# meffmadd/intro-tc-vae

Hardware: AMD Instinct MI355X
Metric: images/sec (64x64x3, z=128, bs=64) intro-TC step (higher is better)
Workload: dtype f32 in/out/accumulate, conv products on split-fp16 MFMA (two scaled fp16 planes, 3 products, fp32-class)

## Files before the change

### intro-tc-vae_amd/csrc/abi.hip

```cpp
#include "conv_shared.h"

#include <vector>

namespace itcv {
thread_local char g_err[512] = "";

struct ProfRec {
  int code;
  double flop;
  hipEvent_t start, stop;
};
static bool g_prof_on = false;
static std::vector<ProfRec> g_prof;

static thread_local int g_prof_depth = 0;
ProfScope::ProfScope(hipStream_t stream, int kind, int ks, int bm, int up2, int ns, double flop) : st(stream), slot(-1) {
  if (++g_prof_depth > 1 || !g_prof_on) return;
  ProfRec r;
  r.code = kind | (ks << 4) | (bm << 8) | (up2 << 16) | (ns << 20);
  r.flop = flop;
  if (hipEventCreate(&r.start) != hipSuccess || hipEventCreate(&r.stop) != hipSuccess) return;
  g_prof.push_back(r);
  slot = (int)g_prof.size() - 1;
  g_prof_start = r.start, g_prof_stop = r.stop;
}
ProfScope::~ProfScope() {
  if (--g_prof_depth > 0) return;
  if (slot >= 0 && g_prof_start) {
    (void)hipEventDestroy(g_prof[slot].start);
    (void)hipEventDestroy(g_prof[slot].stop);
    g_prof.pop_back();
  }
  g_prof_start = g_prof_stop = nullptr;
}
thread_local hipEvent_t g_prof_start = nullptr, g_prof_stop = nullptr;
Options g_opt;
}

extern "C" {
int itcv_abi_version(void) { return ITCV_ABI_VERSION; }

int itcv_set_option(const char* name, int value) {
  if (!name) return itcv::fail("%s: null option name", "itcv_set_option");
  if (!strcmp(name, "band_m16")) {
    if (value != 0 && value != 1) return itcv::fail("%s: band_m16 takes 0 or 1 (got %lld)", "itcv_set_option", value);
    itcv::g_opt.band_m16 = value;
    return 0;
  }
  if (!strcmp(name, "band_persist_blocks")) {
    if (value < 0 || value > 1024) return itcv::fail("%s: band_persist_blocks takes 0..1024 (got %lld)", "itcv_set_option", value);
    itcv::g_opt.band_persist_blocks = value;
    return 0;
  }
  if (!strcmp(name, "wgrad_m16")) {
    if (value != 0 && value != 1) return itcv::fail("%s: wgrad_m16 takes 0 or 1 (got %lld)", "itcv_set_option", value);
    itcv::g_opt.wgrad_m16 = value;
    return 0;
  }
  if (!strcmp(name, "planes_mfma_waves")) {
    if (value != 4 && value != 8) return itcv::fail("%s: planes_mfma_waves takes 4 or 8 (got %lld)", "itcv_set_option", value);
    itcv::g_opt.planes_mfma_waves = value;
    return 0;
  }
  return itcv::fail("%s: unknown option", "itcv_set_option");
}
int itcv_get_option(const char* name) {
  if (name && !strcmp(name, "band_m16")) return itcv::g_opt.band_m16;
  if (name && !strcmp(name, "band_persist_blocks")) return itcv::g_opt.band_persist_blocks;
  if (name && !strcmp(name, "wgrad_m16")) return itcv::g_opt.wgrad_m16;
  if (name && !strcmp(name, "planes_mfma_waves")) return itcv::g_opt.planes_mfma_waves;
  return -1;
}
const char* itcv_last_error(void) { return itcv::g_err; }

int itcv_profile_begin(void) {
  itcv::g_prof.clear();
  itcv::g_prof_on = true;
  return 0;
}
int itcv_profile_end(void) {
  itcv::g_prof_on = false;
  for (auto& r : itcv::g_prof) (void)hipEventSynchronize(r.stop);
  return (int)itcv::g_prof.size();
}
int itcv_profile_get(int i, int* code, double* flop, float* ms) {
  if (i < 0 || i >= (int)itcv::g_prof.size()) return itcv::fail("%s: index out of range", "itcv_profile_get");
  const auto& r = itcv::g_prof[i];
  *code = r.code;
  *flop = r.flop;
  if (hipEventElapsedTime(ms, r.start, r.stop) != hipSuccess) *ms = -1.f;
  return 0;
}
int itcv_profile_clear(void) {
  for (auto& r : itcv::g_prof) {
    (void)hipEventDestroy(r.start);
    (void)hipEventDestroy(r.stop);
  }
  itcv::g_prof.clear();
  return 0;
}
}
```

### intro-tc-vae_amd/csrc/conv_shared.h

```cpp
#pragma once
#include <stdlib.h>

#include "common.h"

namespace itcv {

#ifdef ITCV_DIAG
#define ITCV_ABL(args, bits) (((args).ablate & (bits)) != 0)
#define ITCV_DBG(args) ((args).debug != 0)
static int diag_ablate() {
  static int v = -1;
  if (v < 0) {
    const char* e = getenv("ITCV_ABLATE");
    v = e ? atoi(e) : 0;
  }
  return v;
}
#else
#define ITCV_ABL(args, bits) (false)
#define ITCV_DBG(args) (false)
#endif

typedef float f32x16 __attribute__((ext_vector_type(16)));
typedef float f32x4_t __attribute__((ext_vector_type(4)));
typedef float f32x4 __attribute__((ext_vector_type(4)));

#pragma clang diagnostic ignored "-Winline-asm"
__device__ __forceinline__ void lds_dma16(const void* gptr, uint32_t lds_base) {
  asm volatile("s_mov_b32 m0, %0\n\ts_nop 0\n\tglobal_load_lds_dwordx4 %1, off"
               :
               : "s"(__builtin_amdgcn_readfirstlane(lds_base)), "v"(gptr)
               : "memory", "m0");
}
__device__ __forceinline__ uint32_t lds_addr(const void* p) {
  return (uint32_t)(size_t)(const __attribute__((address_space(3))) void*)p;
}
template <int N>
__device__ __forceinline__ void wait_vmcnt() {
  asm volatile("s_waitcnt vmcnt(%0)" ::"n"(N) : "memory");
}

static inline int log2_exact(int v) {
  if (v <= 0 || (v & (v - 1))) return -1;
  int s = 0;
  while ((1 << s) < v) ++s;
  return s;
}

struct ConvArgsP2 {
  const u32x4* xp;
  const u32x4* wp;
  const float* bias;
  float* y;
  int B, Ci, H, Co;
  int Mp, N;
  int mt, nt;
  int cpt, cpt_per_split;
  int SR, NSEG, NP, NPC, PXB;
  int h_shift;
  float* stats;
  int stat_T;
  const ScaleRec* xscale;
  size_t slab_stride, plane_stride;
#ifdef ITCV_DIAG
  int debug;
#endif
};

__host__ __device__ constexpr int band_taps_per_stage(int bm, int bn, int ) {
  return (bm == 64 || bn == 128) ? 2 : 1;
}

template <bool M16, bool F16 = false>
struct BandMfma;
template <bool F16>
struct BandMfma<false, F16> {
  typedef f32x16 acc_t;
  static constexpr int TS = 32, NR = 16, KSN = 2;
  static __device__ __forceinline__ acc_t mma(bf16x8 a, bf16x8 b, acc_t c) { return mma32x32x16<F16>(a, b, c); }
  static __device__ __forceinline__ int row(int r, int kq) { return (r & 3) + 8 * (r >> 2) + 4 * kq; }
};
template <bool F16>
struct BandMfma<true, F16> {
  typedef float acc_t __attribute__((ext_vector_type(4)));
  static constexpr int TS = 16, NR = 4, KSN = 1;
  static __device__ __forceinline__ acc_t mma(bf16x8 a, bf16x8 b, acc_t c) { return mma16x16x32<F16>(a, b, c); }
  static __device__ __forceinline__ int row(int r, int kq) { return 4 * kq + r; }
};

struct Options {
  int band_m16 = 1;
  int band_persist_blocks = 256;
  int wgrad_m16 = 1;
  int planes_mfma_waves = 8;
};
extern Options g_opt;
inline int band_m16() { return g_opt.band_m16; }

struct FwdPlanP2 {
  int ok, bm, bn, mt, nt, cpt, splits, cps, SR, NSEG, NP, NPC, PXB;
  int rows2;
  size_t lds;
};

FwdPlanP2 plan_fwd_p2(int B, int Ci, int H, int W, int Co, int KS, int ns);
void launch_fwd_p2(const ConvArgsP2& a, const FwdPlanP2& p, int W, int up2, int f16, hipStream_t st);
bool band_is_persistent(const ConvArgsP2& a, const FwdPlanP2& p);

}
```

### intro-tc-vae_amd/csrc/norm_act.hip

```cpp
#include <stdlib.h>

#include "common.h"

namespace itcv {

constexpr int kRedThreads = 256;

__device__ __forceinline__ uint32_t fdiv(uint32_t a, uint32_t d, int sh) { return sh >= 0 ? (a >> sh) : (a / d); }

struct BnGrp {
  size_t xs;
  size_t os;
  size_t dys;
  size_t ps;
  int cs;
  int G;
};

struct BnFinal {
  double count;
  float eps, momentum;
  float* running_mean;
  float* running_var;
  int64_t* nbt;
  float* mean;
  float* rstd;
};

template <bool FUSED>
__global__ __launch_bounds__(kRedThreads) void bn_moments_partial(const float* __restrict__ x,
                                                                  double* __restrict__ part, int B, int C, int HW,
                                                                  int splits, int hw_shift, BnFinal f, BnGrp grp) {
  __shared__ double scratch[kRedThreads / 64];
  const uint32_t c = blockIdx.x, s = blockIdx.y, hw_n = HW, total = (uint32_t)B * hw_n;
  const uint32_t chunk = ((total + splits - 1) / splits + 3) & ~3u;
  const uint32_t beg = s * chunk, end = min(beg + chunk, total);
  const int ngroups = (FUSED && grp.G > 1) ? grp.G : 1;
  if (!FUSED) {
    x += (size_t)blockIdx.z * grp.xs;
    part += (size_t)blockIdx.z * splits * 2 * C;
  }
 for (int gi = 0; gi < ngroups; ++gi, x += grp.xs, f.mean += grp.cs, f.rstd += grp.cs) {
  double s1 = 0.0, s2 = 0.0;
  if ((HW & 3) == 0) {
#pragma unroll 4
    for (uint32_t i = beg + threadIdx.x * 4; i < end; i += kRedThreads * 4) {
      const uint32_t b = fdiv(i, hw_n, hw_shift), hw = i - b * hw_n;
      const float4 v = *reinterpret_cast<const float4*>(x + ((size_t)b * C + c) * hw_n + hw);
      s1 += ((double)v.x + (double)v.y) + ((double)v.z + (double)v.w);
      s2 += ((double)v.x * v.x + (double)v.y * v.y) + ((double)v.z * v.z + (double)v.w * v.w);
    }
  } else {
    for (uint32_t i = beg + threadIdx.x; i < end; i += kRedThreads) {
      const uint32_t b = fdiv(i, hw_n, hw_shift), hw = i - b * hw_n;
      const float v = x[((size_t)b * C + c) * hw_n + hw];
      s1 += (double)v;
      s2 += (double)v * v;
    }
  }
  s1 = block_sum(s1, scratch);
  s2 = block_sum(s2, scratch);
  if (threadIdx.x == 0) {
    if (FUSED) {
      const double m = s1 / f.count;
      double var = s2 / f.count - m * m;
      if (var < 0.0) var = 0.0;
      f.mean[c] = (float)m;
      f.rstd[c] = (float)(1.0 / sqrt(var + (double)f.eps));
      if (f.running_mean) f.running_mean[c] = (1.f - f.momentum) * f.running_mean[c] + f.momentum * (float)m;
      if (f.running_var) {
        const double unbiased = f.count > 1.0 ? var * f.count / (f.count - 1.0) : var;
        f.running_var[c] = (1.f - f.momentum) * f.running_var[c] + f.momentum * (float)unbiased;
      }
      if (c == 0 && f.nbt) f.nbt[0] += 1;
    } else {
      part[((size_t)s * 2 + 0) * C + c] = s1;
      part[((size_t)s * 2 + 1) * C + c] = s2;
    }
  }
 }
}

__global__ void combine_partials(const double* __restrict__ part, double* __restrict__ sums, int C2, int splits) {
  const int i = blockIdx.x * blockDim.x + threadIdx.x;
  if (i >= C2) return;
// ... 254 lines not shown
                if (vg < 0.0) vg = 0.0;
              }
              if (st.running_mean) st.running_mean[c] = (1.f - st.momentum) * st.running_mean[c] + st.momentum * (float)mg;
              if (st.running_var) {
                const double unbiased = st.count > 1.0 ? vg * st.count / (st.count - 1.0) : vg;
                st.running_var[c] = (1.f - st.momentum) * st.running_var[c] + st.momentum * (float)unbiased;
              }
            }
            if (c == 0 && st.nbt) st.nbt[0] += G;
          }
        }
      }
      __syncthreads();
    }
    if (idx >= total) continue;
    const uint32_t bc8 = idx / per_plane, pp = idx - bc8 * per_plane;
    const uint32_t b = bc8 / C8, c8 = bc8 - b * C8;
    float o[8][PX];
    float4 xin[POOL ? 1 : 8];
    float p_ga[8], p_be[8], p_mu[8], p_rs[8];
#pragma unroll
    for (int j = 0; j < 8; ++j) {
      const int c = c8 * 8 + j;
      if (POOL == 0) xin[POOL ? 0 : j] = *reinterpret_cast<const float4*>(x + ((size_t)b * C + c) * HW + (size_t)pp * 4);
      p_ga[j] = gamma[c], p_be[j] = beta[c];
      p_mu[j] = STATS ? s_mean[(bc8 - g0) * 8 + j] : mean[c], p_rs[j] = STATS ? s_rstd[(bc8 - g0) * 8 + j] : rstd[c];
    }
#pragma unroll
    for (int j = 0; j < 8; ++j) {
      const int c = c8 * 8 + j;
      const float mu = p_mu[j], rs = p_rs[j];
      const float sc = p_ga[j] * rs, sh = p_be[j] - mu * sc;
      const size_t bc = (size_t)b * C + c;
      if (POOL == 0) {
        const size_t i = bc * HW + (size_t)pp * 4;
        float4 v = xin[POOL ? 0 : j];
        v.x = v.x * sc + sh, v.y = v.y * sc + sh, v.z = v.z * sc + sh, v.w = v.w * sc + sh;
        if (skip) {
          const float4 k = *reinterpret_cast<const float4*>(skip + i);
          v.x += k.x, v.y += k.y, v.z += k.z, v.w += k.w;
        }
        v.x = lrelu(v.x, slope), v.y = lrelu(v.y, slope), v.z = lrelu(v.z, slope), v.w = lrelu(v.w, slope);
        if (y) *reinterpret_cast<float4*>(y + i) = v;
        o[j][0] = v.x, o[j][1] = v.y, o[j][POOL ? 0 : 2] = v.z, o[j][POOL ? 1 : 3] = v.w;
      } else {
        const uint32_t ho = (pp * 2) / Wo, wo = pp * 2 - ho * Wo;
        const size_t src = bc * HW + (size_t)(2 * ho) * W + 2 * wo;
        const float4 a = *reinterpret_cast<const float4*>(x + src);
        const float4 bb = *reinterpret_cast<const float4*>(x + src + W);
        float v0 = a.x * sc + sh, v1 = a.y * sc + sh, v2 = bb.x * sc + sh, v3 = bb.y * sc + sh;
        float w0 = a.z * sc + sh, w1 = a.w * sc + sh, w2 = bb.z * sc + sh, w3 = bb.w * sc + sh;
        if (skip) {
          const float4 ka = *reinterpret_cast<const float4*>(skip + src);
          const float4 kb = *reinterpret_cast<const float4*>(skip + src + W);
          v0 += ka.x, v1 += ka.y, v2 += kb.x, v3 += kb.y;
          w0 += ka.z, w1 += ka.w, w2 += kb.z, w3 += kb.w;
        }
        const float r0 = 0.25f * (lrelu(v0, slope) + lrelu(v1, slope) + lrelu(v2, slope) + lrelu(v3, slope));
        const float r1 = 0.25f * (lrelu(w0, slope) + lrelu(w1, slope) + lrelu(w2, slope) + lrelu(w3, slope));
        if (y) *reinterpret_cast<float2*>(y + bc * HWo + (size_t)pp * 2) = make_float2(r0, r1);
        o[j][0] = r0, o[j][1] = r1;
      }
    }
    u32x4 chk[PX][NS];
#pragma unroll
    for (int px = 0; px < PX; ++px) {
      float v8[8];
#pragma unroll
      for (int j = 0; j < 8; ++j) v8[j] = o[j][px];
      split8<NS, F16>(v8, chk[px]);
    }
    const uint32_t cidx0 = base + (threadIdx.x & ~63u);
    if (STRIP && cidx0 + 64 <= total) {
      store_planes_wave<PX, NS>(planes, plane_stride, per_plane, (uint32_t)HWo, cidx0, chk, strips[STRIP ? threadIdx.x >> 6 : 0]);
    } else {
#pragma unroll
      for (int px = 0; px < PX; ++px)
#pragma unroll
        for (int p = 0; p < NS; ++p) planes[(size_t)p * plane_stride + (size_t)bc8 * HWo + (size_t)pp * PX + px] = chk[px][p];
    }
  }
}

template <int MODE>
__device__ __forceinline__ float upstream(const float* __restrict__ dy, size_t bc, int h, int w, int H, int W) {
  if (MODE == 0) return dy[bc * H * W + (size_t)h * W + w];
  if (MODE == 1) return 0.25f * dy[bc * (H / 2) * (W / 2) + (size_t)(h >> 1) * (W / 2) + (w >> 1)];
  const size_t base = bc * (size_t)(4 * H * W) + (size_t)(2 * h) * (2 * W) + 2 * w;
  const float2 a = *reinterpret_cast<const float2*>(dy + base);
  const float2 b = *reinterpret_cast<const float2*>(dy + base + 2 * W);
  return (a.x + a.y) + (b.x + b.y);
}

template <int MODE>
__global__ __launch_bounds__(kRedThreads) void bn_bwd_partial(const float* __restrict__ x,
                                                              const float* __restrict__ dy,
                                                              const float* __restrict__ mean,
                                                              const float* __restrict__ rstd,
                                                              const float* __restrict__ gamma,
                                                              const float* __restrict__ beta,
                                                              const float* __restrict__ skip,
                                                              double* __restrict__ part, int B, int C, int H, int W,
                                                              float slope, int splits) {
  __shared__ double scratch[kRedThreads / 64];
  const int c = blockIdx.x, s = blockIdx.y, HW = H * W;
  const size_t total = (size_t)B * HW;
  const size_t chunk = (total + splits - 1) / splits;
  const size_t beg = (size_t)s * chunk, end = beg + chunk < total ? beg + chunk : total;
  const float mu = mean[c], rs = rstd[c], ga = gamma[c], be = beta[c];
  double s1 = 0.0, s2 = 0.0;
  for (size_t i = beg + threadIdx.x; i < end; i += kRedThreads) {
    const size_t b = i / HW;
    const int hw = (int)(i - b * HW), h = hw / W, w = hw - h * W;
    const size_t bc = b * C + c;
    const float xh = (x[bc * HW + hw] - mu) * rs;
    float u = xh * ga + be;
    if (skip) u += skip[bc * HW + hw];
    float g = upstream<MODE>(dy, bc, h, w, H, W);
    if (!(u > 0.f)) g *= slope;
    s1 += (double)g;
    s2 += (double)g * (double)xh;
  }
  s1 = block_sum(s1, scratch);
  s2 = block_sum(s2, scratch);
  if (threadIdx.x == 0) {
    part[((size_t)s * 2 + 0) * C + c] = s1;
    part[((size_t)s * 2 + 1) * C + c] = s2;
  }
}

template <int MODE>
__global__ void bn_bwd_apply_kernel(const float* __restrict__ x, const float* __restrict__ dy,
                                    const float* __restrict__ mean, const float* __restrict__ rstd,
                                    const float* __restrict__ gamma, const float* __restrict__ beta,
                                    const float* __restrict__ skip, const double* __restrict__ dsums, double count,
                                    float* __restrict__ dx, float* __restrict__ dskip, int C, int H, int W,
                                    size_t n, float slope) {
  const int HW = H * W;
  for (size_t i = (size_t)blockIdx.x * blockDim.x + threadIdx.x; i < n; i += (size_t)gridDim.x * blockDim.x) {
    const size_t bc = i / HW;
    const int hw = (int)(i - bc * HW), h = hw / W, w = hw - h * W;
    const int c = (int)(bc % C);
    const float mu = mean[c], rs = rstd[c], ga = gamma[c];
    const float xh = (x[i] - mu) * rs;
    float u = xh * ga + beta[c];
    if (skip) u += skip[i];
    float g = upstream<MODE>(dy, bc, h, w, H, W);
    if (!(u > 0.f)) g *= slope;
    const float m1 = (float)(dsums[c] / count), m2 = (float)(dsums[C + c] / count);
    dx[i] = ga * rs * (g - m1 - xh * m2);
    if (dskip) dskip[i] = g;
  }
}



template <int MODE>
__device__ __forceinline__ float4 upstream4(const float* __restrict__ dy, uint32_t bc, uint32_t h, uint32_t w,
                                            uint32_t H, uint32_t W) {
  if (MODE == 0) return *reinterpret_cast<const float4*>(dy + (size_t)bc * H * W + h * W + w);
  if (MODE == 1) {
    const float2 d = *reinterpret_cast<const float2*>(dy + (size_t)bc * (H / 2) * (W / 2) + (h >> 1) * (W / 2) + (w >> 1));
    return make_float4(0.25f * d.x, 0.25f * d.x, 0.25f * d.y, 0.25f * d.y);
  }
  const float* p = dy + (size_t)bc * (4 * H * W) + (size_t)(2 * h) * (2 * W) + 2 * w;
  const float4 a0 = *reinterpret_cast<const float4*>(p), a1 = *reinterpret_cast<const float4*>(p + 4);
// ... 563 lines not shown
    ITCV_BWD_PARTIAL(1);
  else if (up2)
    ITCV_BWD_PARTIAL(2);
  else
    ITCV_BWD_PARTIAL(0);
#undef ITCV_BWD_PARTIAL
  ITCV_CHECK_LAUNCH("itcv_bn_act_bwd_reduce");
  if (vec && splits == 1) return 0;
  hipLaunchKernelGGL(bn_combine_param_kernel, dim3(cdiv(C, 256)), dim3(256), 0, S(stream), part, dsums, C, splits,
                     dgamma, dbeta, accumulate);
  ITCV_CHECK_LAUNCH("itcv_bn_act_bwd_reduce(combine)");
  return 0;
}

static int bwd_apply_impl(const float* x, const float* dy, const float* mean, const float* rstd, const float* gamma,
                          const float* beta, const float* skip, const double* dsums, const double* local_dsums,
                          double count, float* dx, float* dskip, float* dgamma, float* dbeta, int accumulate, int B,
                          int C, int H, int W, float slope, int pool, int up2, void* dx_planes, int ns,
                          size_t plane_stride, const float* mx, int nmx, void* stream) {
  ITCV_REQUIRE(x && dy && mean && rstd && gamma && beta && dsums && (dx || dx_planes) && B > 0 && C > 0 && count > 0,
               "itcv_bn_act_bwd_apply");
  const size_t pstride = plane_stride ? plane_stride : (size_t)B * (C / 8) * H * W;
  ITCV_REQUIRE(!(pool && up2), "itcv_bn_act_bwd_apply(pool and up2 are exclusive)");
  const size_t n = (size_t)B * C * H * W;
  const bool vec = (W % 4 == 0) && (n < (1ull << 31));
  const int wsh = ilog2_exact(W), hwsh = ilog2_exact(H * W), cmask = ilog2_exact(C) >= 0 ? C - 1 : -1;
  hipStream_t st = S(stream);
  if (dx_planes) {
    ITCV_REQUIRE(bn_fmt_ok(ns) && vec && itcv_bn_act_planes_supported(C, H, W, 0), "itcv_bn_act_bwd_apply(planes)");
    if (ns == ITCV_PLANES_F16X2 && !mx)
      return fail("%s: fp16 gradient planes take their scale from the maxima of the reduce pass: use itcv_bn_train_bwd",
                  "itcv_bn_act_bwd_apply");
    const dim3 grid(grid_for(n / 32)), blk(256);
    u32x4* pl = static_cast<u32x4*>(dx_planes);
#define ITCV_BWD_PLANES(MODE_, NS_, F_)                                                                          \
  do {                                                                                                           \
      launch_timed((bn_bwd_apply_planes<MODE_, NS_, false, true, F_>), grid, blk, 0, st, x, dy, mean, rstd, gamma, beta, \
                         skip, dsums, count, dx, dskip, pl, B, C, H, W, slope, wsh, BnBwdSumsIn{}, pstride, BnGrp{}, mx, nmx); \
  } while (0)
#define ITCV_BWD_PLANES_NS(MODE_)                                   \
  do {                                                              \
    if (ns == ITCV_PLANES_F16X2) ITCV_BWD_PLANES(MODE_, 2, true);   \
    else if (ns == 2) ITCV_BWD_PLANES(MODE_, 2, false);             \
    else ITCV_BWD_PLANES(MODE_, 3, false);                          \
  } while (0)
    if (pool) ITCV_BWD_PLANES_NS(1);
    else if (up2) ITCV_BWD_PLANES_NS(2);
    else ITCV_BWD_PLANES_NS(0);
#undef ITCV_BWD_PLANES_NS
#undef ITCV_BWD_PLANES
    ITCV_CHECK_LAUNCH("itcv_bn_act_bwd_apply(planes)");
    if (dgamma || dbeta) {
      hipLaunchKernelGGL(bn_param_grad_kernel, dim3(cdiv(C, 256)), dim3(256), 0, st, local_dsums ? local_dsums : dsums,
                         dgamma, dbeta, C, accumulate);
      ITCV_CHECK_LAUNCH("itcv_bn_act_bwd_apply(param grads)");
    }
    return 0;
  }
#define ITCV_BWD_APPLY(MODE)                                                                                      \
  do {                                                                                                            \
    if (vec)                                                                                                      \
      hipLaunchKernelGGL(bn_bwd_apply_v4<MODE>, dim3(grid_for(n, 4)), dim3(256), 0, st, x, dy, mean, rstd, gamma,  \
                         beta, skip, dsums, count, dx, dskip, C, H, W, (uint32_t)(n / 4), slope, wsh, hwsh, cmask); \
    else                                                                                                          \
      hipLaunchKernelGGL(bn_bwd_apply_kernel<MODE>, dim3(grid_for(n)), dim3(256), 0, st, x, dy, mean, rstd, gamma, \
                         beta, skip, dsums, count, dx, dskip, C, H, W, n, slope);                                 \
  } while (0)
  if (pool)
    ITCV_BWD_APPLY(1);
  else if (up2)
    ITCV_BWD_APPLY(2);
  else
    ITCV_BWD_APPLY(0);
#undef ITCV_BWD_APPLY
  ITCV_CHECK_LAUNCH("itcv_bn_act_bwd_apply");
  if (dgamma || dbeta) {
    hipLaunchKernelGGL(bn_param_grad_kernel, dim3(cdiv(C, 256)), dim3(256), 0, S(stream),
                       local_dsums ? local_dsums : dsums, dgamma, dbeta, C, accumulate);
    ITCV_CHECK_LAUNCH("itcv_bn_act_bwd_apply(param grads)");
  }
  return 0;
}

extern "C" {
int itcv_bn_act_bwd_reduce(const float* x, const float* dy, const float* mean, const float* rstd, const float* gamma,
                           const float* beta, const float* skip, double* dsums, float* dgamma, float* dbeta,
                           int accumulate, int B, int C, int H, int W, float slope, int pool, int up2, void* ws,
                           size_t ws_bytes, void* stream) {
  return bwd_reduce_impl(x, dy, mean, rstd, gamma, beta, skip, dsums, dgamma, dbeta, accumulate, B, C, H, W, slope, pool, up2,
                         ws, ws_bytes, nullptr, stream);
}
int itcv_bn_act_bwd_apply(const float* x, const float* dy, const float* mean, const float* rstd, const float* gamma,
                          const float* beta, const float* skip, const double* dsums, const double* local_dsums,
                          double count, float* dx, float* dskip, float* dgamma, float* dbeta, int accumulate, int B,
                          int C, int H, int W, float slope, int pool, int up2, void* dx_planes, int ns,
                          size_t plane_stride, void* stream) {
  return bwd_apply_impl(x, dy, mean, rstd, gamma, beta, skip, dsums, local_dsums, count, dx, dskip, dgamma, dbeta, accumulate,
                        B, C, H, W, slope, pool, up2, dx_planes, ns, plane_stride, nullptr, 0, stream);
}

int itcv_bn_train_fwd(const float* x, const float* gamma, const float* beta, const float* skip, float* y, void* planes,
                      int ns, int B, int C, int H, int W, float slope, int pool, float eps, float momentum,
                      float* running_mean, float* running_var, int64_t* num_batches_tracked, float* mean, float* rstd,
                      void* ws, size_t ws_bytes, size_t plane_stride, const float* tile_stats, int tiles, int tile_pitch,
                      int groups, void* stream) {
  ITCV_REQUIRE(x && gamma && beta && mean && rstd && (y || planes) && B > 0 && C > 0 && H > 0 && W > 0, "itcv_bn_train_fwd");
  const double px_out = (double)(groups > 1 ? groups : 1) * B * C * (pool ? H * W / 4 : H * W);
  ProfScope bn_prof(S(stream), 13, ilog2_exact(W) >= 0 ? ilog2_exact(W) : 0, C / 8, pool ? 1 : 0, planes ? ns : 0,
                    (double)(groups > 1 ? groups : 1) * B * C * H * W * 4.0 * (skip ? 2 : 1) + px_out * ((planes ? 4.0 : 0.0) + (y ? 4.0 : 0.0)));
  if (groups > 1) {
    ITCV_REQUIRE(!planes || plane_stride, "itcv_bn_train_fwd(groups need the plane stride of the whole tensor)");
    const int HWg = H * W, HWo = pool ? HWg / 4 : HWg;
    const size_t xs = (size_t)B * C * HWg, os = (size_t)B * C * HWo, ps = (size_t)B * (C / 8) * HWo;
    const int gsplits = bn_splits(B, C, HWg);
    const bool mergeable = !tile_stats && planes && bn_fmt_ok(ns) && itcv_bn_act_planes_supported(C, H, W, pool) &&
                           xs < (1ull << 31);
    const bool merged = mergeable && gsplits == 1;
    if (mergeable && gsplits > 1 && ws && ws_bytes >= (size_t)groups * gsplits * 2 * C * sizeof(double)) {
      const BnGrp grp{xs, os, 0, ps, C, groups};
      double* part = static_cast<double*>(ws);
      hipLaunchKernelGGL(bn_moments_partial<false>, dim3(C, gsplits, groups), dim3(kRedThreads), 0, S(stream), x, part, B, C,
                         HWg, gsplits, ilog2_exact(HWg), BnFinal{}, grp);
      ITCV_CHECK_LAUNCH("itcv_bn_train_fwd(grouped partials)");
      const int per_plane_g = pool ? (HWg / 4) / 2 : HWg / 4;
      const bool fold_in_apply = per_plane_g >= 64;
      if (!fold_in_apply) {
        hipLaunchKernelGGL(bn_combine_finalize_groups_kernel, dim3(cdiv(C, 256)), dim3(256), 0, S(stream), part, gsplits,
                           groups, (double)B * HWg, eps, momentum, running_mean, running_var, num_batches_tracked, mean, rstd,
                           C);
        ITCV_CHECK_LAUNCH("itcv_bn_train_fwd(grouped finalize)");
      }
      const BnStatsIn stg{part, gsplits, (double)B * HWg, eps, momentum, running_mean, running_var, num_batches_tracked, mean,
                          rstd};
      const size_t threads = (size_t)B * (C / 8) * (HWo / (pool ? 2 : 4));
      const dim3 grid(grid_for(threads), 1, groups), blk(256);
      u32x4* pl = static_cast<u32x4*>(planes);
#define ITCV_FWD_GRP2_K(POOL_, NS_, ST_, F_)                                                                              \
  launch_timed((bn_act_fwd_planes_kernel<POOL_, NS_, ST_, true, F_>), grid, blk, 0, S(stream), x, mean, rstd, gamma, beta, \
                     skip, y, pl, B, C, H, W, slope, (ST_) ? stg : BnStatsIn{}, plane_stride, grp)
#define ITCV_FWD_GRP2(POOL_, NS_, F_)                                  \
  do {                                                                 \
    if (fold_in_apply) ITCV_FWD_GRP2_K(POOL_, NS_, true, F_);          \
    else ITCV_FWD_GRP2_K(POOL_, NS_, false, F_);                       \
  } while (0)
#define ITCV_FWD_GRP2_NS(POOL_)                                     \
  do {                                                              \
    if (ns == ITCV_PLANES_F16X2) ITCV_FWD_GRP2(POOL_, 2, true);     \
    else if (ns == 2) ITCV_FWD_GRP2(POOL_, 2, false);               \
    else ITCV_FWD_GRP2(POOL_, 3, false);                            \
  } while (0)
      if (pool) ITCV_FWD_GRP2_NS(1);
      else ITCV_FWD_GRP2_NS(0);
#undef ITCV_FWD_GRP2_NS
#undef ITCV_FWD_GRP2_K
#undef ITCV_FWD_GRP2
      ITCV_CHECK_LAUNCH("itcv_bn_train_fwd(grouped apply)");
      return 0;
    }
    if (!merged) {
      for (int g = 0; g < groups; ++g)
        if (int e = itcv_bn_train_fwd(x + g * xs, gamma, beta, skip ? skip + g * xs : nullptr, y ? y + g * os : nullptr,
                                      planes ? static_cast<u32x4*>(planes) + g * ps : nullptr, ns, B, C, H, W, slope, pool,
                                      eps, momentum, running_mean, running_var, num_batches_tracked, mean + (size_t)g * C,
                                      rstd + (size_t)g * C, ws, ws_bytes, plane_stride,
                                      tile_stats ? tile_stats + (size_t)g * tiles : nullptr, tiles, tile_pitch, 1, stream))
          return e;
      return 0;
    }
    const BnGrp grp{xs, os, 0, ps, C, groups};
    const BnFinal f{(double)B * HWg, eps, momentum, running_mean, running_var, num_batches_tracked, mean, rstd};
    hipLaunchKernelGGL(bn_moments_partial<true>, dim3(C, 1), dim3(kRedThreads), 0, S(stream), x, static_cast<double*>(nullptr),
                       B, C, HWg, 1, ilog2_exact(HWg), f, grp);
    ITCV_CHECK_LAUNCH("itcv_bn_train_fwd(grouped statistics)");
    const size_t threads = (size_t)B * (C / 8) * (HWo / (pool ? 2 : 4));
    const dim3 grid(grid_for(threads), 1, groups), blk(256);
    u32x4* pl = static_cast<u32x4*>(planes);
#define ITCV_FWD_GRP(POOL_, NS_, F_)                                                                                      \
  do {                                                                                                                    \
      launch_timed((bn_act_fwd_planes_kernel<POOL_, NS_, false, true, F_>), grid, blk, 0, S(stream), x, mean, rstd, gamma, \
                         beta, skip, y, pl, B, C, H, W, slope, BnStatsIn{}, plane_stride, grp);                             \
  } while (0)
#define ITCV_FWD_GRP_NS(POOL_)                                     \
  do {                                                             \
    if (ns == ITCV_PLANES_F16X2) ITCV_FWD_GRP(POOL_, 2, true);     \
    else if (ns == 2) ITCV_FWD_GRP(POOL_, 2, false);               \
    else ITCV_FWD_GRP(POOL_, 3, false);                            \
  } while (0)
    if (pool) ITCV_FWD_GRP_NS(1);
    else ITCV_FWD_GRP_NS(0);
#undef ITCV_FWD_GRP_NS
#undef ITCV_FWD_GRP
    ITCV_CHECK_LAUNCH("itcv_bn_train_fwd(grouped apply)");
    return 0;
  }
  const size_t pstride = plane_stride ? plane_stride : (size_t)B * (C / 8) * (pool ? (H / 2) * (W / 2) : H * W);
  if (tile_stats) {
    ITCV_REQUIRE(tiles > 0 && tile_pitch >= tiles, "itcv_bn_train_fwd(tile statistics)");
    hipLaunchKernelGGL(bn_tile_stats_finalize_kernel, dim3(C), dim3(256), 0, S(stream), tile_stats, tiles, tile_pitch,
                       (double)B * H * W, eps, momentum, running_mean, running_var, num_batches_tracked, mean, rstd, C);
    ITCV_CHECK_LAUNCH("itcv_bn_train_fwd(tile statistics)");
    return itcv_bn_act_fwd(x, mean, rstd, gamma, beta, skip, y, B, C, H, W, slope, pool, planes, ns, plane_stride, stream);
  }
  const int HW = H * W, splits = bn_splits(B, C, HW);
  const int per_plane = pool ? (HW / 4) / 2 : HW / 4;
  const bool fusable = planes && bn_fmt_ok(ns) && itcv_bn_act_planes_supported(C, H, W, pool) && splits > 1 &&
                       per_plane >= 64 && (size_t)B * C * HW < (1ull << 31);
  if (!fusable) {
    if (int e = itcv_bn_train_stats(x, B, C, HW, eps, momentum, running_mean, running_var, num_batches_tracked, mean,
                                    rstd, ws, ws_bytes, stream))
      return e;
    return itcv_bn_act_fwd(x, mean, rstd, gamma, beta, skip, y, B, C, H, W, slope, pool, planes, ns, plane_stride, stream);
  }
  ITCV_REQUIRE(ws && ws_bytes >= (size_t)splits * 2 * C * sizeof(double), "itcv_bn_train_fwd(workspace)");
  double* part = static_cast<double*>(ws);
  hipLaunchKernelGGL(bn_moments_partial<false>, dim3(C, splits), dim3(kRedThreads), 0, S(stream), x, part, B, C, HW,
                     splits, ilog2_exact(HW), BnFinal{}, BnGrp{});
  ITCV_CHECK_LAUNCH("itcv_bn_train_fwd(partials)");
  const BnStatsIn st{part, splits, (double)B * HW, eps, momentum, running_mean, running_var, num_batches_tracked, mean, rstd};
  const size_t threads = (size_t)B * (C / 8) * per_plane;
  const dim3 grid(grid_for(threads)), blk(256);
  u32x4* pl = static_cast<u32x4*>(planes);
#define ITCV_FWD_FUSED(POOL_, NS_, F_)                                                                               \
  do {                                                                                                                \
      launch_timed((bn_act_fwd_planes_kernel<POOL_, NS_, true, true, F_>), grid, blk, 0, S(stream), x, mean, rstd, gamma, \
                         beta, skip, y, pl, B, C, H, W, slope, st, pstride, BnGrp{});                                            \
  } while (0)
#define ITCV_FWD_FUSED_NS(POOL_)                                     \
  do {                                                               \
    if (ns == ITCV_PLANES_F16X2) ITCV_FWD_FUSED(POOL_, 2, true);     \
    else if (ns == 2) ITCV_FWD_FUSED(POOL_, 2, false);               \
    else ITCV_FWD_FUSED(POOL_, 3, false);                            \
  } while (0)
  if (pool) ITCV_FWD_FUSED_NS(1);
  else ITCV_FWD_FUSED_NS(0);
#undef ITCV_FWD_FUSED_NS
#undef ITCV_FWD_FUSED
  ITCV_CHECK_LAUNCH("itcv_bn_train_fwd(apply)");
  return 0;
}

int itcv_bn_train_bwd(const float* x, const float* dy, const float* mean, const float* rstd, const float* gamma,
                      const float* beta, const float* skip, double* dsums, float* dx, float* dskip, void* dx_planes,
                      int ns, float* dgamma, float* dbeta, int accumulate, int B, int C, int H, int W, float slope,
                      int pool, int up2, void* ws, size_t ws_bytes, size_t plane_stride, int groups, void* stream) {
  ITCV_REQUIRE(x && dy && mean && rstd && gamma && beta && dsums && (dx || dx_planes) && B > 0 && C > 0,
               "itcv_bn_train_bwd");
  ITCV_REQUIRE(!(pool && up2), "itcv_bn_train_bwd(pool and up2 are exclusive)");
  const double bn_el = (double)(groups > 1 ? groups : 1) * B * C * H * W;
  ProfScope bn_prof(S(stream), 14, ilog2_exact(W) >= 0 ? ilog2_exact(W) : 0, C / 8, pool ? 1 : (up2 ? 2 : 0), dx_planes ? ns : 0,
                    bn_el * 4.0 * (1.0 + (pool ? 0.25 : (up2 ? 4.0 : 1.0)) + (skip ? 1.0 : 0.0)) +
                        bn_el * ((dx_planes ? 4.0 : 0.0) + (dx ? 4.0 : 0.0) + (dskip ? 4.0 : 0.0)));
  if (groups > 1) {
    ITCV_REQUIRE(!dx_planes || plane_stride, "itcv_bn_train_bwd(groups need the plane stride of the whole tensor)");
    const int HWg = H * W;
    const size_t xs = (size_t)B * C * HWg, dys = pool ? xs / 4 : (up2 ? xs * 4 : xs), ps = (size_t)B * (C / 8) * HWg;
    const bool vecg = (W % 4 == 0) && xs < (1ull << 31);
    const int gsplits = bn_splits(B, C, HWg);
    const bool mergeable = vecg && dx_planes && bn_fmt_ok(ns) && itcv_bn_act_planes_supported(C, H, W, 0);
    const bool merged = mergeable && gsplits == 1;
    const bool f16 = ns == ITCV_PLANES_F16X2;
    const int nmx = groups * gsplits * C;
    const size_t ws_need = (size_t)groups * gsplits * 2 * C * sizeof(double) + (f16 ? (size_t)2 * nmx * sizeof(float) : 0);
    float* mx = f16 && ws ? reinterpret_cast<float*>(static_cast<double*>(ws) + (size_t)groups * gsplits * 2 * C) : nullptr;
    if (f16 && !(mergeable && ws && ws_bytes >= ws_need))
      return fail("%s: fp16 gradient planes need the merged group path (W %% 4 == 0, planes, a workspace of itcv_bn_workspace * groups)",
                  "itcv_bn_train_bwd");
    if (mergeable && gsplits > 1 && ws && ws_bytes >= ws_need) {
      if (pool) ITCV_REQUIRE(H % 2 == 0 && W % 2 == 0, "itcv_bn_train_bwd(pool)");
      const BnGrp grp{xs, 0, dys, ps, C, groups};
      hipStream_t st = S(stream);
      const int wsh = ilog2_exact(W), hwsh = ilog2_exact(HWg);
      double* part = static_cast<double*>(ws);
      const dim3 rgrid(C, gsplits, groups), agrid(grid_for(xs / 32), 1, groups), blk(256);
      u32x4* pl = static_cast<u32x4*>(dx_planes);
      const double count = (double)B * HWg;
      const bool fold_in_apply = HWg / 4 >= 64;
      const BnBwdSumsIn smg{part, gsplits, dsums, dgamma, dbeta, accumulate};
#define ITCV_BWD_GRP2_K(MODE_, NS_, SUMS_, F_)                                                                           \
  launch_timed((bn_bwd_apply_planes<MODE_, NS_, SUMS_, true, F_>), agrid, blk, 0, st, x, dy, mean, rstd, gamma, beta, \
                     skip, (SUMS_) ? static_cast<const double*>(nullptr) : dsums, count, dx, dskip, pl, B, C, H, W, slope, \
                     wsh, (SUMS_) ? smg : BnBwdSumsIn{}, plane_stride, grp, mx, nmx)
#define ITCV_BWD_GRP2(MODE_, NS_, F_)                                                                                    \
  do {                                                                                                                   \
    hipLaunchKernelGGL((bn_bwd_partial_v4<MODE_, false, F_>), rgrid, dim3(kRedThreads), 0, st, x, dy, mean, rstd, gamma, beta, \
                       skip, part, B, C, H, W, slope, gsplits, wsh, hwsh, BnBwdFinal{}, grp, mx, nmx);                   \
    if (fold_in_apply) {                                                                                                 \
// ... 163 lines not shown
```

Baseline: 3911.

## Fuse BN-train statistics, finalize and activation apply into one launch for small maps

```diff
diff --git a/intro-tc-vae_amd/csrc/abi.hip b/intro-tc-vae_amd/csrc/abi.hip
--- a/intro-tc-vae_amd/csrc/abi.hip
+++ b/intro-tc-vae_amd/csrc/abi.hip
@@ -62,6 +62,11 @@
     itcv::g_opt.planes_mfma_waves = value;
     return 0;
   }
+  if (!strcmp(name, "bn_fwd_onelaunch")) {
+    if (value != 0 && value != 1) return itcv::fail("%s: bn_fwd_onelaunch takes 0 or 1 (got %lld)", "itcv_set_option", value);
+    itcv::g_opt.bn_fwd_onelaunch = value;
+    return 0;
+  }
   return itcv::fail("%s: unknown option", "itcv_set_option");
 }
 int itcv_get_option(const char* name) {
@@ -69,6 +74,7 @@
   if (name && !strcmp(name, "band_persist_blocks")) return itcv::g_opt.band_persist_blocks;
   if (name && !strcmp(name, "wgrad_m16")) return itcv::g_opt.wgrad_m16;
   if (name && !strcmp(name, "planes_mfma_waves")) return itcv::g_opt.planes_mfma_waves;
+  if (name && !strcmp(name, "bn_fwd_onelaunch")) return itcv::g_opt.bn_fwd_onelaunch;
   return -1;
 }
 const char* itcv_last_error(void) { return itcv::g_err; }
diff --git a/intro-tc-vae_amd/csrc/conv_shared.h b/intro-tc-vae_amd/csrc/conv_shared.h
--- a/intro-tc-vae_amd/csrc/conv_shared.h
+++ b/intro-tc-vae_amd/csrc/conv_shared.h
@@ -93,6 +93,7 @@
   int band_persist_blocks = 256;
   int wgrad_m16 = 1;
   int planes_mfma_waves = 8;
+  int bn_fwd_onelaunch = 1;
 };
 extern Options g_opt;
 inline int band_m16() { return g_opt.band_m16; }
diff --git a/intro-tc-vae_amd/csrc/norm_act.hip b/intro-tc-vae_amd/csrc/norm_act.hip
--- a/intro-tc-vae_amd/csrc/norm_act.hip
+++ b/intro-tc-vae_amd/csrc/norm_act.hip
@@ -1,6 +1,7 @@
 #include <stdlib.h>
 
 #include "common.h"
+#include "conv_shared.h"
 
 namespace itcv {
 
@@ -421,6 +422,142 @@
   }
 }
 
+constexpr int kOneLaunchPerChannel = 1024;
+
+template <int POOL, int NS, bool F16>
+__global__ __launch_bounds__(kRedThreads) void bn_fwd_onelaunch_kernel(
+    const float* __restrict__ x, const float* __restrict__ gamma, const float* __restrict__ beta,
+    const float* __restrict__ skip, float* __restrict__ y, u32x4* __restrict__ planes, int B, int C, int H, int W,
+    float slope, int hw_shift, BnFinal f, size_t plane_stride, BnGrp grp) {
+  if constexpr (F16) {
+    if (blockIdx.x == 0 && threadIdx.x == 0) {
+      ScaleRec* rec = reinterpret_cast<ScaleRec*>(planes + (size_t)NS * plane_stride);
+      rec->scale = 1.f, rec->inv = 1.f, rec->pad[0] = rec->pad[1] = 0.f;
+    }
+  }
+  __shared__ double scratch[16][kRedThreads / 64];
+  __shared__ float s_mean[8], s_rstd[8];
+  constexpr int PX = POOL ? 2 : 4;
+  const uint32_t c8 = blockIdx.x, hw_n = H * W, total = (uint32_t)B * hw_n;
+  const int HW = H * W, C8 = C >> 3;
+  const int Ho = POOL ? H / 2 : H, Wo = POOL ? W / 2 : W, HWo = Ho * Wo;
+  const uint32_t per_plane = (uint32_t)HWo / PX, items = (uint32_t)B * per_plane;
+  const int ngroups = grp.G > 1 ? grp.G : 1;
+  for (int gi = 0; gi < ngroups; ++gi, x += grp.xs, f.mean += grp.cs, f.rstd += grp.cs) {
+    double s[16];
+#pragma unroll
+    for (int k = 0; k < 16; ++k) s[k] = 0.0;
+#pragma unroll 2
+    for (uint32_t i = threadIdx.x * 4; i < total; i += kRedThreads * 4) {
+      const uint32_t b = fdiv(i, hw_n, hw_shift), hw = i - b * hw_n;
+      float4 v[8];
+#pragma unroll
+      for (int j = 0; j < 8; ++j) v[j] = *reinterpret_cast<const float4*>(x + ((size_t)b * C + c8 * 8 + j) * hw_n + hw);
+#pragma unroll
+      for (int j = 0; j < 8; ++j) {
+        s[j] += ((double)v[j].x + (double)v[j].y) + ((double)v[j].z + (double)v[j].w);
+        s[8 + j] += ((double)v[j].x * v[j].x + (double)v[j].y * v[j].y) + ((double)v[j].z * v[j].z + (double)v[j].w * v[j].w);
+      }
+    }
+#pragma unroll
+    for (int k = 0; k < 16; ++k) s[k] = wave_sum(s[k]);
+    __syncthreads();
+    if ((threadIdx.x & 63) == 0) {
+#pragma unroll
+      for (int k = 0; k < 16; ++k) scratch[k][threadIdx.x >> 6] = s[k];
+    }
+    __syncthreads();
+    if (threadIdx.x < 8) {
+      const int j = threadIdx.x, c = c8 * 8 + j;
+      double s1 = 0, s2 = 0;
+      for (int i = 0; i < kRedThreads / 64; ++i) s1 += scratch[j][i];
+      for (int i = 0; i < kRedThreads / 64; ++i) s2 += scratch[8 + j][i];
+      const double m = s1 / f.count;
+      double var = s2 / f.count - m * m;
+      if (var < 0.0) var = 0.0;
+      const float mf = (float)m, rf = (float)(1.0 / sqrt(var + (double)f.eps));
+      f.mean[c] = mf;
+      f.rstd[c] = rf;
+      s_mean[j] = mf, s_rstd[j] = rf;
+      if (f.running_mean) f.running_mean[c] = (1.f - f.momentum) * f.running_mean[c] + f.momentum * (float)m;
+      if (f.running_var) {
+        const double unbiased = f.count > 1.0 ? var * f.count / (f.count - 1.0) : var;
+        f.running_var[c] = (1.f - f.momentum) * f.running_var[c] + f.momentum * (float)unbiased;
+      }
+      if (c == 0 && f.nbt) f.nbt[0] += 1;
+    }
+    __syncthreads();
+    const float* xg = x;
+    const float* kg = skip ? skip + gi * grp.xs : nullptr;
+    float* yg = y ? y + gi * grp.os : nullptr;
+    u32x4* pg = NS ? planes + gi * grp.ps : nullptr;
+    for (uint32_t idx = threadIdx.x; idx < items; idx += kRedThreads) {
+      const uint32_t b = idx / per_plane, pp = idx - b * per_plane;
+      const uint32_t bc8 = b * C8 + c8;
+      float o[8][PX];
+      float4 xin[POOL ? 1 : 8];
+      float p_ga[8], p_be[8], p_mu[8], p_rs[8];
+#pragma unroll
+      for (int j = 0; j < 8; ++j) {
+        const int c = c8 * 8 + j;
+        if (POOL == 0) xin[POOL ? 0 : j] = *reinterpret_cast<const float4*>(xg + ((size_t)b * C + c) * HW + (size_t)pp * 4);
+        p_ga[j] = gamma[c], p_be[j] = beta[c];
+        p_mu[j] = s_mean[j], p_rs[j] = s_rstd[j];
+      }
+#pragma unroll
+      for (int j = 0; j < 8; ++j) {
+        const int c = c8 * 8 + j;
+        const float mu = p_mu[j], rs = p_rs[j];
+        const float sc = p_ga[j] * rs, sh = p_be[j] - mu * sc;
+        const size_t bc = (size_t)b * C + c;
+        if (POOL == 0) {
+          const size_t i = bc * HW + (size_t)pp * 4;
+          float4 v = xin[POOL ? 0 : j];
+          v.x = v.x * sc + sh, v.y = v.y * sc + sh, v.z = v.z * sc + sh, v.w = v.w * sc + sh;
+          if (kg) {
+            const float4 k = *reinterpret_cast<const float4*>(kg + i);
+            v.x += k.x, v.y += k.y, v.z += k.z, v.w += k.w;
+          }
+          v.x = lrelu(v.x, slope), v.y = lrelu(v.y, slope), v.z = lrelu(v.z, slope), v.w = lrelu(v.w, slope);
+          if (yg) *reinterpret_cast<float4*>(yg + i) = v;
+          o[j][0] = v.x, o[j][1] = v.y, o[j][POOL ? 0 : 2] = v.z, o[j][POOL ? 1 : 3] = v.w;
+        } else {
+          const uint32_t ho = (pp * 2) / Wo, wo = pp * 2 - ho * Wo;
+          const size_t src = bc * HW + (size_t)(2 * ho) * W + 2 * wo;
+          const float4 a = *reinterpret_cast<const float4*>(xg + src);
+          const float4 bb = *reinterpret_cast<const float4*>(xg + src + W);
+          float v0 = a.x * sc + sh, v1 = a.y * sc + sh, v2 = bb.x * sc + sh, v3 = bb.y * sc + sh;
+          float w0 = a.z * sc + sh, w1 = a.w * sc + sh, w2 = bb.z * sc + sh, w3 = bb.w * sc + sh;
+          if (kg) {
+            const float4 ka = *reinterpret_cast<const float4*>(kg + src);
+            const float4 kb = *reinterpret_cast<const float4*>(kg + src + W);
+            v0 += ka.x, v1 += ka.y, v2 += kb.x, v3 += kb.y;
+            w0 += ka.z, w1 += ka.w, w2 += kb.z, w3 += kb.w;
+          }
+          const float r0 = 0.25f * (lrelu(v0, slope) + lrelu(v1, slope) + lrelu(v2, slope) + lrelu(v3, slope));
+          const float r1 = 0.25f * (lrelu(w0, slope) + lrelu(w1, slope) + lrelu(w2, slope) + lrelu(w3, slope));
+          if (yg) *reinterpret_cast<float2*>(yg + bc * HWo + (size_t)pp * 2) = make_float2(r0, r1);
+          o[j][0] = r0, o[j][1] = r1;
+        }
+      }
+      if constexpr (NS > 0) {
+        u32x4 chk[PX][NS];
+#pragma unroll
+        for (int px = 0; px < PX; ++px) {
+          float v8[8];
+#pragma unroll
+          for (int j = 0; j < 8; ++j) v8[j] = o[j][px];
+          split8<NS, F16>(v8, chk[px]);
+        }
+#pragma unroll
+        for (int px = 0; px < PX; ++px)
+#pragma unroll
+          for (int p = 0; p < NS; ++p) pg[(size_t)p * plane_stride + (size_t)bc8 * HWo + (size_t)pp * PX + px] = chk[px][p];
+      }
+    }
+  }
+}
+
 template <int MODE>
 __device__ __forceinline__ float upstream(const float* __restrict__ dy, size_t bc, int h, int w, int H, int W) {
   if (MODE == 0) return dy[bc * H * W + (size_t)h * W + w];
@@ -1150,6 +1287,32 @@
   return 0;
 }
 
+static bool bn_fwd_onelaunch(const float* x, const float* gamma, const float* beta, const float* skip, float* y,
+                             void* planes, int ns, int B, int C, int H, int W, float slope, int pool, const BnFinal& f,
+                             size_t plane_stride, const BnGrp& grp, hipStream_t st) {
+  const int HW = H * W, G = grp.G > 1 ? grp.G : 1;
+  if (!g_opt.bn_fwd_onelaunch || !itcv_bn_act_planes_supported(C, H, W, pool) || (planes && !bn_fmt_ok(ns)) ||
+      bn_splits(B, C, HW) != 1 || (size_t)B * HW > (size_t)kOneLaunchPerChannel ||
+      (size_t)G * B * C * HW >= (1ull << 31))
+    return false;
+  u32x4* pl = static_cast<u32x4*>(planes);
+#define ITCV_FWD_ONE(POOL_, NS_, F_)                                                                                    \
+  launch_timed((bn_fwd_onelaunch_kernel<POOL_, NS_, F_>), dim3(C / 8), dim3(kRedThreads), 0, st, x, gamma, beta, skip, y, \
+               pl, B, C, H, W, slope, ilog2_exact(HW), f, plane_stride, grp)
+#define ITCV_FWD_ONE_NS(POOL_)                                       \
+  do {                                                               \
+    if (!planes) ITCV_FWD_ONE(POOL_, 0, false);                      \
+    else if (ns == ITCV_PLANES_F16X2) ITCV_FWD_ONE(POOL_, 2, true);  \
+    else if (ns == 2) ITCV_FWD_ONE(POOL_, 2, false);                 \
+    else ITCV_FWD_ONE(POOL_, 3, false);                              \
+  } while (0)
+  if (pool) ITCV_FWD_ONE_NS(1);
+  else ITCV_FWD_ONE_NS(0);
+#undef ITCV_FWD_ONE_NS
+#undef ITCV_FWD_ONE
+  return true;
+}
+
 extern "C" {
 int itcv_bn_act_bwd_reduce(const float* x, const float* dy, const float* mean, const float* rstd, const float* gamma,
                            const float* beta, const float* skip, double* dsums, float* dgamma, float* dbeta,
@@ -1181,6 +1344,13 @@
     const int HWg = H * W, HWo = pool ? HWg / 4 : HWg;
     const size_t xs = (size_t)B * C * HWg, os = (size_t)B * C * HWo, ps = (size_t)B * (C / 8) * HWo;
     const int gsplits = bn_splits(B, C, HWg);
+    if (!tile_stats && gsplits == 1 &&
+        bn_fwd_onelaunch(x, gamma, beta, skip, y, planes, ns, B, C, H, W, slope, pool,
+                         BnFinal{(double)B * HWg, eps, momentum, running_mean, running_var, num_batches_tracked, mean, rstd},
+                         plane_stride, BnGrp{xs, os, 0, ps, C, groups}, S(stream))) {
+      ITCV_CHECK_LAUNCH("itcv_bn_train_fwd(grouped, one launch)");
+      return 0;
+    }
     const bool mergeable = !tile_stats && planes && bn_fmt_ok(ns) && itcv_bn_act_planes_supported(C, H, W, pool) &&
                            xs < (1ull << 31);
     const bool merged = mergeable && gsplits == 1;
@@ -1270,6 +1440,13 @@
     return itcv_bn_act_fwd(x, mean, rstd, gamma, beta, skip, y, B, C, H, W, slope, pool, planes, ns, plane_stride, stream);
   }
   const int HW = H * W, splits = bn_splits(B, C, HW);
+  if (splits == 1 &&
+      bn_fwd_onelaunch(x, gamma, beta, skip, y, planes, ns, B, C, H, W, slope, pool,
+                       BnFinal{(double)B * HW, eps, momentum, running_mean, running_var, num_batches_tracked, mean, rstd},
+                       pstride, BnGrp{}, S(stream))) {
+    ITCV_CHECK_LAUNCH("itcv_bn_train_fwd(one launch)");
+    return 0;
+  }
   const int per_plane = pool ? (HW / 4) / 2 : HW / 4;
   const bool fusable = planes && bn_fmt_ok(ns) && itcv_bn_act_planes_supported(C, H, W, pool) && splits > 1 &&
                        per_plane >= 64 && (size_t)B * C * HW < (1ull << 31);
```

Result: no change. 3898, median of 6 (-0.3%).
